# Liufeiran123/qwen2-audio-whisper-ggml

Measured on AMD Instinct MI355X. Metric: encoder audio-frames/sec (30 s clips) at 1/2/4/8 MI355X; MFMA util %, higher is better.
Workload: dtype q4_k x q8_k integer dots on fp16 MFMA (fp32 acc); 1 GPU; configs[2]: batch=64 30 s clips, Q4_K quantized weights, 1xMI355X per rank; model=qwen2-audio-encoder L32 D1280 H20 F5120 (synthetic weights), weights=q4_k, clips_per_gpu=64, global_batch=64, seq_len=3000, parallelism=dp1

## Files before the change

### include/q2a_encoder.h

```cpp
#ifndef Q2A_ENCODER_H
#define Q2A_ENCODER_H

#include <stddef.h>
#include <stdint.h>

#ifdef __cplusplus
extern "C" {
#endif

typedef struct q2a_engine q2a_engine;

typedef enum {
    Q2A_OK = 0,
    Q2A_ERR_IO = -1,
    Q2A_ERR_FORMAT = -2,
    Q2A_ERR_HIP = -3,
    Q2A_ERR_ARG = -4,
    Q2A_ERR_OOM = -5,
    Q2A_ERR_UNSUPPORTED = -6
} q2a_status;

#define Q2A_CLIP_ENCODED 0
#define Q2A_CLIP_SKIPPED 1
#define Q2A_CLIP_FAILED 2
// ... 66 lines not shown
                          int n_clips, int offset_ms, float * out_host, int32_t * status);
int q2a_group_setup_times(const q2a_group * g, double * pack_s, double * broadcast_s, double * open_s, int64_t * blob_bytes);

enum {
    Q2A_PROF_MEL = 0, Q2A_PROF_CONV1, Q2A_PROF_CONV2, Q2A_PROF_LN, Q2A_PROF_GEMM_QKV, Q2A_PROF_ATTN,
    Q2A_PROF_QUANT, Q2A_PROF_GEMM_O, Q2A_PROF_GEMM_FC1, Q2A_PROF_GEMM_FC2, Q2A_PROF_POOL, Q2A_PROF_CLASSES
};
int q2a_profile_enable(q2a_engine * e, int on);
int q2a_profile_enable_mask(q2a_engine * e, unsigned mask);
int q2a_profile_read(q2a_engine * e, double * ms, int64_t * counts, int n, int reset);

int q2a_test_linear(q2a_engine * e, int layer, int which, const float * x_dev, int M, float * y_dev, void * stream);
int q2a_test_block(q2a_engine * e, int layer, float * x_dev, int n_clips, void * stream);
int q2a_test_block_taps(q2a_engine * e, int layer, float * x_dev, int n_clips, void * const * taps, void * stream);
int q2a_test_frontend(q2a_engine * e, const float * pcm_dev, int64_t pcm_stride, const int32_t * n_samples, int n_clips,
                      float * x_dev, void * stream);
int q2a_test_pool_ln(q2a_engine * e, const float * x_dev, int n_clips, float * out_dev, void * stream);
int q2a_test_fc1_path(q2a_engine * e, int path);
int q2a_test_attention(q2a_engine * e, const float * q_dev, const float * k_dev, const float * v_dev, int n_clips,
                       float * out_dev, void * stream);
int q2a_test_attention_len(q2a_engine * e, const float * q_dev, const float * k_dev, const float * v_dev, int n_clips,
                           const int32_t * key_len, float * out_dev, void * stream);
int q2a_test_block_len(q2a_engine * e, int layer, float * x_dev, int n_clips, const int32_t * key_len, void * stream);

typedef struct q2a_projector q2a_projector;
q2a_projector * q2a_projector_open(const char * path, int device);
void q2a_projector_close(q2a_projector * p);
int q2a_projector_get_dims(const q2a_projector * p, int * d_in, int * d_out, int * wtype);
int q2a_projector_apply(q2a_projector * p, const float * x_dev, int64_t rows, float * y_dev, void * stream);

#ifdef __cplusplus
}
#endif
#endif
```

### qwen2-audio-whisper-ggml_amd/csrc/q2a_attn.hip

```cpp
#include "q2a_internal.h"

#include <cstddef>
#include <cstdlib>
#include <cstring>

namespace {

typedef _Float16 half8 __attribute__((ext_vector_type(8)));
typedef _Float16 half4 __attribute__((ext_vector_type(4)));
typedef short short8_t __attribute__((ext_vector_type(8)));
typedef float f16v __attribute__((ext_vector_type(16)));
typedef float f4v_t __attribute__((ext_vector_type(4)));
typedef __bf16 bf8 __attribute__((ext_vector_type(8)));
typedef __attribute__((address_space(3))) void * lds_ptr_t;

template <bool BF>
__device__ __forceinline__ f16v mma32(half8 a, half8 b, f16v c) {
    if constexpr (BF) return __builtin_amdgcn_mfma_f32_32x32x16_bf16(__builtin_bit_cast(bf8, a), __builtin_bit_cast(bf8, b), c, 0, 0, 0);
    else return __builtin_amdgcn_mfma_f32_32x32x16_f16(a, b, c, 0, 0, 0);
}
template <bool BF>
__device__ __forceinline__ _Float16 to16(float v) {
    if constexpr (BF) return __builtin_bit_cast(_Float16, (__bf16) v);
    else return (_Float16) v;
}


constexpr int KT = 64;
template <bool SW> struct attn_lds;
template <> struct attn_lds<false> {
    static constexpr int KROW = 144, VROW = 136;
    static __device__ __forceinline__ int k(int, int ch) { return ch << 4; }
    static __device__ __forceinline__ int v(int, int c8) { return c8 << 3; }
};
template <> struct attn_lds<true> {
// ... 27 lines not shown
}
constexpr int KS = 32;
__device__ __forceinline__ half2_t rem_pair(float p0, float p1, half2_t h) {
    half2_t r;
    asm("v_fma_mixlo_f16 %0, %1, -1.0, %2 op_sel_hi:[1,0,0]" : "=v"(r) : "v"(h), "v"(p0));
    asm("v_fma_mixhi_f16 %0, %1, -1.0, %2 op_sel:[1,0,0] op_sel_hi:[1,0,0]" : "+v"(r) : "v"(h), "v"(p1));
    return r;
}
__device__ __forceinline__ f4v_t mma16(half8 a, half8 b, f4v_t c) {
    return __builtin_amdgcn_mfma_f32_16x16x32_f16(a, b, c, 0, 0, 0);
}
__device__ __forceinline__ float max_lane16(float x) {
    const auto r = __builtin_amdgcn_permlane16_swap(__float_as_uint(x), __float_as_uint(x), false, false);
    return fmaxf(__uint_as_float(r[0]), __uint_as_float(r[1]));
}
__device__ __forceinline__ float sum_lane16(float x) {
    const auto r = __builtin_amdgcn_permlane16_swap(__float_as_uint(x), __float_as_uint(x), false, false);
    return __uint_as_float(r[0]) + __uint_as_float(r[1]);
}
__device__ __forceinline__ float sum_lane32(float x) {
    const auto r = __builtin_amdgcn_permlane32_swap(__float_as_uint(x), __float_as_uint(x), false, false);
    return __uint_as_float(r[0]) + __uint_as_float(r[1]);
}
template <bool VR, int NQB, bool KL = false>
__global__ __launch_bounds__(256, 3) void k_attn_t(const q2a_attn_args p) {
    static_assert(NQB == 1 || NQB == 2, "16 or 32 queries per wave");
    static_assert(!KL || VR, "key lengths: row-major V only (the V^T image's columns are not clamped)");
    constexpr int QWG = 64 * NQB;
    constexpr int KROW = 128, VROW = 64;
    constexpr int KIMG = KS * KROW, VIMG = 64 * VROW;
    constexpr int STAGE = 2 * KIMG + 2 * VIMG;
    __shared__ __attribute__((aligned(16))) char ldsA[STAGE];
    __shared__ __attribute__((aligned(16))) char ldsB[STAGE];
    __shared__ __attribute__((aligned(16))) char ldsC[STAGE];
    const int tid = threadIdx.x, lane = tid & 63, wave = __builtin_amdgcn_readfirstlane(tid >> 6);
    const int T = p.T, D = p.D;
    const int nq = (T + QWG - 1) / QWG, total = (int) gridDim.x;
    const int L = (int) blockIdx.x;
    const int w = (total & 7) ? L : (L & 7) * (total >> 3) + (L >> 3);
    const int qt = w % nq, h = (w / nq) % p.H, clip = w / (nq * p.H);
    const int q0 = qt * QWG + wave * 16 * NQB;
    const int64_t rowbase = (int64_t) clip * T;
    const int c16 = lane & 15, g = lane >> 4;
    int Tk = T;
    if constexpr (KL) {
        Tk = min(max(p.key_len[clip], 1), T);
        if (qt * QWG >= Tk) {
#pragma unroll
            for (int qb = 0; qb < NQB; ++qb) {
                const int q = q0 + 16 * qb + c16;
// ... 288 lines not shown
        for (int qb = 0; qb < NQB; ++qb) rebase(s0, qb, true);
        exps(s0, ex);
        splat(init);
    }
    for (int t = 0; t < ntiles; t += 3) {
        iter(ldsB, ldsA, ldsC, t);
        if (t + 1 >= ntiles) break;
        iter(ldsC, ldsB, ldsA, t + 1);
        if (t + 2 >= ntiles) break;
        iter(ldsA, ldsC, ldsB, t + 2);
    }

#pragma unroll
    for (int qb = 0; qb < NQB; ++qb) {
        const float l_tot = sum_lane32(sum_lane16(l_run[qb]));
        const float inv = 1.0f / l_tot;
        const int q = q0 + 16 * qb + c16;
        if (q < T) {
            const int64_t orow = (rowbase + q) * D + h * 64;
#pragma unroll
            for (int db = 0; db < 4; ++db) {
                const int d = 16 * db + 4 * g;
                f4v_t v = o[qb][db] * inv;
                if (p.outH) {
                    asm volatile("" : "+v"(v));
                    const half4 hv = {(_Float16) v[0], (_Float16) v[1], (_Float16) v[2], (_Float16) v[3]};
                    *(half4 *) (p.outH + orow + d) = hv;
                } else {
                    *(float4 *) (p.outF + orow + d) = make_float4(v[0], v[1], v[2], v[3]);
                }
            }
        }
    }
}

template <bool BF>
__global__ __launch_bounds__(512, 2) void k_attn_pp(const q2a_attn_args p) {
    constexpr float QL2E = BF ? L2E : 1.0f;
    typedef attn_lds<false> LY;
    constexpr int KROW = LY::KROW, VROW = LY::KROW;
    constexpr int KIMG = KT * KROW, VIMG = 64 * VROW;
    constexpr int NK = BF ? 1 : 2;
    constexpr int STAGE = NK * KIMG + VIMG;
    constexpr int NST = 3;
    constexpr int CH = (NK + 1) * 512;
    constexpr int CPT = CH / 512;
    __shared__ __attribute__((aligned(16))) char lds[NST * STAGE];
    const int tid = threadIdx.x, lane = tid & 63, wave = tid >> 6;
    const int grp = wave >> 2, gt = tid & 255;
    const int T = p.T, D = p.D;
    const int nq = (T + 255) / 256, total = (int) gridDim.x;
    const int L = (int) blockIdx.x;
    const int w = (total & 7) ? L : (L & 7) * (total >> 3) + (L >> 3);
    const int qt = w % nq, h = (w / nq) % p.H, clip = w / (nq * p.H);
    const int q0 = qt * 256 + wave * 32;
// ... 186 lines not shown
                    *(half4 *) (p.outH + orow + d) = hv;
                } else {
                    *(float4 *) (p.outF + orow + d) = make_float4(v0, v1, v2, v3);
                }
            }
    }
}
}

bool q2a_attention_wants_vlo() { return true; }

#ifndef Q2A_ATTN_LAUNCH
#define Q2A_ATTN_LAUNCH q2a_launch_attention
#endif
namespace {
hipError_t launch_attention(const q2a_attn_args & a, hipStream_t s) {
    if (a.D != a.H * 64 || a.TP < ((a.T + KT - 1) / KT) * KT) return hipErrorInvalidValue;
    if (a.key_len && (a.bf16 || !a.v_rows)) return hipErrorInvalidValue;
    if (a.bf16) {
        if (!a.outH) return hipErrorInvalidValue;
        hipLaunchKernelGGL(k_attn_pp<true>, dim3(((a.T + 255) / 256) * a.H * a.n_clips), dim3(512), 0, s, a);
    } else {
        if (!a.vtl) return hipErrorInvalidValue;
        const int n2 = ((a.T + 127) / 128) * a.H * a.n_clips;
        const bool narrow = n2 < q2a_cu_count();
        const dim3 grid(narrow ? ((a.T + 63) / 64) * a.H * a.n_clips : n2);
        if (a.key_len) {
            if (narrow) hipLaunchKernelGGL((k_attn_t<true, 1, true>), grid, dim3(256), 0, s, a);
            else hipLaunchKernelGGL((k_attn_t<true, 2, true>), grid, dim3(256), 0, s, a);
        } else if (a.v_rows) {
            if (narrow) hipLaunchKernelGGL((k_attn_t<true, 1>), grid, dim3(256), 0, s, a);
            else hipLaunchKernelGGL((k_attn_t<true, 2>), grid, dim3(256), 0, s, a);
        } else {
            if (narrow) hipLaunchKernelGGL((k_attn_t<false, 1>), grid, dim3(256), 0, s, a);
            else hipLaunchKernelGGL((k_attn_t<false, 2>), grid, dim3(256), 0, s, a);
        }
    }
    return hipGetLastError();
}
}

hipError_t Q2A_ATTN_LAUNCH(const q2a_attn_args & a, hipStream_t s) {
    q2a_attn_args b;
    memcpy(&b, &a, offsetof(q2a_attn_args, key_len));
    b.key_len = nullptr;
    return launch_attention(b, s);
}

hipError_t q2a_launch_attention_len(const q2a_attn_args & a, hipStream_t s) { return launch_attention(a, s); }
```

### qwen2-audio-whisper-ggml_amd/csrc/q2a_engine.hip

```cpp
#include "q2a_encoder.h"
#include "q2a_format.h"
#include "q2a_internal.h"

#include <algorithm>
#include <cmath>
#include <cerrno>
#include <cstdarg>
#include <cstdio>
#include <cstdlib>
#include <cstring>
#include <string>
#include <thread>
#include <vector>

namespace {

thread_local std::string g_err;

void set_err(const char * fmt, ...) {
    char buf[512];
    va_list ap;
    va_start(ap, fmt);
    vsnprintf(buf, sizeof(buf), fmt, ap);
    va_end(ap);
// ... 650 lines not shown
        size_t in_cap = 0, out_cap = 0;
        hipEvent_t h2d = nullptr, comp = nullptr, d2h = nullptr;
    };
    hipStream_t copy_stream = nullptr;
    host_buf hb[2];
    float * out_stage = nullptr;
    int32_t * meta = nullptr;
    int32_t * meta_host = nullptr;
    hipEvent_t meta_evt = nullptr;
    float * mel = nullptr;
    q2a_half * xc1 = nullptr;
    q2a_half * y1 = nullptr;
    float * X = nullptr;
    q2a_half * actD = nullptr;
    q2a_half * actF = nullptr;
    float * dyD = nullptr;
    float * dyF = nullptr;
    q2a_half * aextD = nullptr;
    q2a_half * aextF = nullptr;
    q2a_half *qh = nullptr, *ql = nullptr, *kh = nullptr, *kl = nullptr, *vt = nullptr;
    q2a_half * vtl = nullptr;
    float * attF = nullptr;
    float * hF = nullptr;
    float * part = nullptr;
    int2 * frange = nullptr;
    int TP = 0;
    int dy_ld = 0;
    bool force_encode = false;
    int fc1_path = 0;
    void * taps[4] = {nullptr, nullptr, nullptr, nullptr};

    bool prof = false;
    struct rec { int cls; hipEvent_t a, b; };
    std::vector<rec> pending;
    std::vector<hipEvent_t> pool;
    unsigned prof_mask = ~0u;
    double prof_ms[Q2A_PROF_CLASSES] = {};
    int64_t prof_n[Q2A_PROF_CLASSES] = {};

    template <class P> P g(int i) const { return (P) (blob + h.goff[i]); }
    template <class P> P lv(int l, int i) const { return (P) (blob + h.loff[l][i]); }
    const uint64_t * mat(int l, int w) const { return h.loff[l] + L_MAT0 + w * A_COUNT; }
};

namespace {

inline hipStream_t call_stream(const void * stream) { return (hipStream_t) stream; }

int engine_init(q2a_engine * e, int device) {
    int n = 0;
    HIP_TRY(hipGetDeviceCount(&n));
    if (device < 0 || device >= n) { set_err("device %d not available (%d devices)", device, n); return Q2A_ERR_HIP; }
    e->device = device;
    HIP_TRY(hipSetDevice(device));
    HIP_TRY(hipStreamCreateWithFlags(&e->stream, hipStreamNonBlocking));
    HIP_TRY(hipEventCreateWithFlags(&e->meta_evt, hipEventDisableTiming));
    return Q2A_OK;
}

int engine_adopt_header(q2a_engine * e) {
    if (const char * why = header_problem(e->h)) { set_err("%s", why); return Q2A_ERR_FORMAT; }
    e->d = dims_of(e->h.hp);
    e->wtype = e->h.wtype;
    e->blk = e->h.blk;
    e->f32 = e->wtype == Q2A_TYPE_F32;
    e->bf16 = e->h.act == Q2A_ACT_BF16;
    e->kx = e->f32 && !e->bf16 ? 3 : 1;
    e->gblk = e->bf16 ? Q2A_BLK_BF16 : e->blk;
    e->TP = ((e->d.T + 63) / 64) * 64;
    return Q2A_OK;
}

void free_ws(q2a_engine * e) {
    if (e->ws) (void) hipFree(e->ws);
    if (e->meta_host) (void) hipHostFree(e->meta_host);
    e->ws = nullptr; e->meta_host = nullptr;
    e->cap_clips = 0; e->ws_bytes = 0;
}

// ... 49 lines not shown
    HIP_TRY(hipSetDevice(e->device));
    HIP_TRY(hipDeviceSynchronize());
    if (e->ws) { (void) hipFree(e->ws); e->ws = nullptr; }
    if (e->meta_host) { (void) hipHostFree(e->meta_host); e->meta_host = nullptr; }
    const dims & d = e->d;
    const int64_t BT = (int64_t) B * d.T;
    const bool quant = e->blk != 0;
    size_t off = 0;
    auto take = [&](size_t bytes) { const size_t o = off; off += (bytes + 255) & ~size_t(255); return o; };
    const size_t o_meta = take((size_t) B * 5 * 4);
    const size_t o_mel = take((size_t) B * d.M * d.TM * 4);
    const size_t o_xc1 = take((size_t) B * (d.TM + 2) * 3 * d.M * 2);
    const size_t o_y1 = take((size_t) B * (d.TM + 1) * d.D * 2 * (e->f32 ? 2 : 1));
    const size_t o_X = take((size_t) BT * d.D * 4);
    const size_t o_actD = take((size_t) BT * d.D * 2 * e->kx);
    const size_t o_actF = take((size_t) BT * d.F * 2 * e->kx);
    const size_t o_qh = take((size_t) BT * d.D * 2);
    const size_t o_ql = take((size_t) BT * d.D * 2);
    const size_t o_kh = take((size_t) BT * d.D * 2);
    const size_t o_kl = take((size_t) BT * d.D * 2);
    const size_t o_vt = take((size_t) B * d.H * 64 * e->TP * 2);
    const bool vlo = !e->bf16 && q2a_attention_wants_vlo();
    const size_t o_vtl = vlo ? take((size_t) B * d.H * 64 * e->TP * 2) : 0;
    size_t o_dyD = 0, o_dyF = 0, o_aD = 0, o_aF = 0, o_att = 0, o_hF = 0, o_part = 0;
    const int64_t split_rows = std::min<int64_t>(BT, 32768);
    const bool split = !q2a_gemm_wide_tiles((int) split_rows, d.D, e->gblk);
    if (split) o_part = take((size_t) 4 * split_rows * d.D * 4);
    const int64_t MP = (BT + 255) / 256 * 256;
    e->dy_ld = (int) MP;
    if (quant) {
        o_dyD = take((size_t) MP * (d.D / 32) * 4);
        o_dyF = take((size_t) MP * (d.F / 32) * 4);
        o_aD = take((size_t) MP * (d.D / 256 + 1) * 16 * 2);
        o_aF = take((size_t) MP * (d.F / 256 + 1) * 16 * 2);
        o_att = take((size_t) BT * d.D * 4);
        o_hF = take((size_t) BT * d.F * 4);
    } else if (e->f32) {
        o_att = take((size_t) BT * d.D * 4);
    }
    void * ws = nullptr;
    if (hipMalloc(&ws, off) != hipSuccess) {
        (void) hipGetLastError();
        set_err("workspace allocation of %.2f GB for %d clips failed", off / 1e9, B);
        return Q2A_ERR_OOM;
    }
    HIP_TRY(hipMemsetAsync(ws, 0, off, e->stream));
    HIP_TRY(hipHostMalloc((void **) &e->meta_host, (size_t) B * 5 * 4, hipHostMallocDefault));
    uint8_t * b = (uint8_t *) ws;
    e->ws = ws; e->ws_bytes = off; e->cap_clips = B;
    e->meta = (int32_t *) (b + o_meta);
    e->mel = (float *) (b + o_mel);
    e->xc1 = (q2a_half *) (b + o_xc1);
    e->y1 = (q2a_half *) (b + o_y1);
    e->X = (float *) (b + o_X);
    e->actD = (q2a_half *) (b + o_actD);
    e->actF = (q2a_half *) (b + o_actF);
    e->qh = (q2a_half *) (b + o_qh); e->ql = (q2a_half *) (b + o_ql);
    e->kh = (q2a_half *) (b + o_kh); e->kl = (q2a_half *) (b + o_kl);
    e->vt = (q2a_half *) (b + o_vt);
    e->vtl = vlo ? (q2a_half *) (b + o_vtl) : nullptr;
    e->part = split ? (float *) (b + o_part) : nullptr;
    if (quant) {
        e->dyD = (float *) (b + o_dyD); e->dyF = (float *) (b + o_dyF);
        e->aextD = (q2a_half *) (b + o_aD); e->aextF = (q2a_half *) (b + o_aF);
        e->attF = (float *) (b + o_att); e->hF = (float *) (b + o_hF);
    } else if (e->f32) {
        e->attF = (float *) (b + o_att);
    }
    HIP_TRY(hipStreamSynchronize(e->stream));
    return Q2A_OK;
}

q2a_gemm_args gemm_base(const q2a_engine * e, int l, int which, const q2a_half * A, int M) {
    q2a_gemm_args a;
    memset(&a, 0, sizeof(a));
    int N, K;
    mat_dims(e->d, which, N, K);
    const uint64_t * m = e->mat(l, which);
    a.A = A; a.lda = (int64_t) K * e->kx; a.a_rpg = M; a.a_gstride = 0; a.a_step = 1;
    a.W = (const q2a_half *) (e->blob + m[A_W]); a.ldw = (int64_t) K * e->kx;
    a.M = M; a.N = N; a.K = K * e->kx;
    a.gelu_tab = e->g<const uint16_t *>(G_GELU);
    a.gelu_c = e->g<const uint16_t *>(G_GELU_C);
    a.T = e->d.T; a.D = e->d.D; a.H = e->d.H; a.TP = e->TP;
    if (e->blk) {
        a.nblk = K / e->blk;
        a.dx = (const float *) (e->blob + m[A_DX]);
        a.dy = K == e->d.D ? e->dyD : e->dyF;
// ... 20 lines not shown
    do {                                                                              \
        q2a_engine::rec r_{cls, nullptr, nullptr};                                    \
        const bool on_ = (e)->prof && (((e)->prof_mask >> (cls)) & 1);                 \
        if (on_) { r_.a = prof_event(e); r_.b = prof_event(e); (void) hipEventRecord(r_.a, s); } \
        hipError_t e_ = (call);                                                       \
        if (e_ != hipSuccess) {                                                       \
            set_err("%s: %s", #call, hipGetErrorString(e_));                        \
            return Q2A_ERR_HIP;                                                       \
        }                                                                             \
        if (on_) { (void) hipEventRecord(r_.b, s); (e)->pending.push_back(r_); }      \
    } while (0)

int ln_mode(const q2a_engine * e) { return e->bf16 ? 4 : e->f32 ? 3 : e->blk == 0 ? 0 : e->blk == 256 ? 1 : 2; }

#define LAUNCH(x)                                                                     \
    do {                                                                              \
        hipError_t e_ = (x);                                                          \
        if (e_ != hipSuccess) {                                                       \
            set_err("%s: %s", #x, hipGetErrorString(e_));                           \
            return Q2A_ERR_HIP;                                                       \
        }                                                                             \
    } while (0)

int run_block(q2a_engine * e, int l, int B, hipStream_t s, const int32_t * key_len = nullptr) {
    const dims & d = e->d;
    const int M = B * d.T;
    const int mode = ln_mode(e);
    auto tap = [&](int i, const q2a_half * src, int K) -> hipError_t {
        if (!e->taps[i]) return hipSuccess;
        return hipMemcpyAsync(e->taps[i], src, (size_t) M * K * e->kx * 2, hipMemcpyDeviceToDevice, s);
    };
    q2a_ln_args ln{e->X, M, d.D, e->lv<const float *>(l, L_LN1W), e->lv<const float *>(l, L_LN1B), mode, e->actD, e->dyD, e->aextD, e->dy_ld};
    PLAUNCH(e, s, Q2A_PROF_LN, q2a_launch_layernorm(ln, s));
    LAUNCH(tap(0, e->actD, d.D));
    {
        q2a_gemm_args a = gemm_base(e, l, 0, e->actD, M);
        a.bias = e->lv<const float *>(l, L_BQKV);
        a.qh = e->qh; a.ql = e->ql; a.kh = e->kh; a.kl = e->kl; a.vt = e->vt; a.vtl = e->vtl;
        a.v_rows = e->bf16 ? 0 : 1;
        a.qscale = (1.0f / sqrtf((float) (d.D / d.H))) * (e->bf16 ? 1.0f : Q2A_LOG2E);
        PLAUNCH(e, s, Q2A_PROF_GEMM_QKV, q2a_launch_gemm(a, Q2A_EPI_QKV, e->gblk, s));
    }
    {
        q2a_attn_args at{e->qh, e->ql, e->kh, e->kl, e->vt, B, d.T, d.D, d.H, e->TP, nullptr, nullptr, e->bf16 ? 1 : 0};
        at.vtl = e->vtl;
        at.v_rows = e->bf16 ? 0 : 1;
        at.key_len = key_len;
        if (mode == 0 || mode == 4) at.outH = e->actD; else at.outF = e->attF;
        if (key_len) PLAUNCH(e, s, Q2A_PROF_ATTN, q2a_launch_attention_len(at, s));
        else PLAUNCH(e, s, Q2A_PROF_ATTN, q2a_launch_attention(at, s));
        if (mode == 3) {
            const int64_t n = (int64_t) M * d.D;
            PLAUNCH(e, s, Q2A_PROF_QUANT, launch_split3(e->attF, e->actD, d.D, n, s));
        } else if (mode == 1 || mode == 2) {
            q2a_quant_args qa{e->attF, nullptr, M, d.D, mode, e->actD, e->dyD, e->aextD, e->dy_ld};
            PLAUNCH(e, s, Q2A_PROF_QUANT, q2a_launch_quant_act(qa, s));
        }
    }
    LAUNCH(tap(1, e->actD, d.D));
    {
        q2a_gemm_args a = gemm_base(e, l, 1, e->actD, M);
        a.bias = e->lv<const float *>(l, L_BO);
        a.outF = e->X; a.ldo = d.D;
        a.part = e->part; a.split_stride = (int64_t) M * d.D;
        PLAUNCH(e, s, Q2A_PROF_GEMM_O, q2a_launch_gemm(a, Q2A_EPI_RESID, e->gblk, s));
    }
    q2a_ln_args ln2{e->X, M, d.D, e->lv<const float *>(l, L_LN2W), e->lv<const float *>(l, L_LN2B), mode, e->actD, e->dyD, e->aextD, e->dy_ld};
    PLAUNCH(e, s, Q2A_PROF_LN, q2a_launch_layernorm(ln2, s));
    LAUNCH(tap(2, e->actD, d.D));
    {
        q2a_gemm_args a = gemm_base(e, l, 2, e->actD, M);
        a.bias = e->lv<const float *>(l, L_B1);
        if (mode == 0 || mode == 3 || mode == 4) {
            a.outH = e->actF; a.ldo = (int64_t) d.F * e->kx; a.o_rpg = M; a.o_gstride = 0; a.o_off = 0;
            a.o_dup = mode == 3 ? 2 * d.F : 0;
            PLAUNCH(e, s, Q2A_PROF_GEMM_FC1, q2a_launch_gemm(a, Q2A_EPI_GELU_H, e->gblk, s));
        } else if (mode == 1 && q2a_gemm_wide_tiles(M, d.F, e->blk) &&
// ... 676 lines not shown
    const int64_t n = (int64_t) n_clips * d.T * d.D;
    const dim3 g((unsigned) ((n + 255) / 256)), b(256);
    hipLaunchKernelGGL(k_split_hilo, g, b, 0, s, q, e->qh, e->ql, n, Q2A_LOG2E);
    hipLaunchKernelGGL(k_split_hilo, g, b, 0, s, k, e->kh, e->kl, n, 1.0f);
    hipLaunchKernelGGL(k_split_hilo, g, b, 0, s, v, e->vt, e->vtl, n, 1.0f);
    LAUNCH(hipGetLastError());
    q2a_attn_args at{e->qh, e->ql, e->kh, e->kl, e->vt, n_clips, d.T, d.D, d.H, e->TP, nullptr, out};
    at.vtl = e->vtl;
    at.v_rows = 1;
    at.key_len = with_len ? e->meta + 4 * n_clips : nullptr;
    if (with_len) LAUNCH(q2a_launch_attention_len(at, s));
    else LAUNCH(q2a_launch_attention(at, s));
    return Q2A_OK;
}

int q2a_test_attention(q2a_engine * e, const float * q, const float * k, const float * v, int n_clips, float * out,
                       void * stream) {
    return test_attention_impl(e, q, k, v, n_clips, nullptr, false, out, stream);
}

int q2a_test_attention_len(q2a_engine * e, const float * q, const float * k, const float * v, int n_clips,
                           const int32_t * key_len, float * out, void * stream) {
    return test_attention_impl(e, q, k, v, n_clips, key_len, true, out, stream);
}

struct q2a_projector {
    int device = 0;
    hipStream_t stream = nullptr;
    int d_in = 0, d_out = 0, wtype = 0, blk = 0;
    void * wdev = nullptr;
    uint64_t off[A_COUNT] = {};
    float * bias = nullptr;
    void * ws = nullptr;
    size_t ws_bytes = 0;
    const uint16_t * gelu = nullptr;
};

q2a_projector * q2a_projector_open(const char * path, int device) {
    char err[256] = {0};
    q2a_model_file * mf = q2a_model_file_read(path, err, sizeof(err));
    if (!mf) { set_err("projector %s: %s", path ? path : "(null)", err); return nullptr; }
    const q2a_tensor_desc * wt = q2a_model_file_find(mf, "multi_modal_projector.linear.weight");
    const q2a_tensor_desc * bt = q2a_model_file_find(mf, "multi_modal_projector.linear.bias");
    auto fail = [&](int code, const char * msg) -> q2a_projector * {
        set_err("projector %s: %s", path, msg);
        q2a_model_file_free(mf);
// ... 108 lines not shown
```

### qwen2-audio-whisper-ggml_amd/csrc/q2a_internal.h

```cpp
#pragma once

#include <hip/hip_runtime.h>
#include <stdint.h>

typedef _Float16 q2a_half;

extern "C" void q2a_internal_set_error(const char * msg);
struct q2a_engine;
extern "C" int q2a_internal_engine_blob(const q2a_engine * e, const void ** blob, int64_t * bytes, int * device);

enum q2a_epi {
    Q2A_EPI_QKV = 0,
    Q2A_EPI_RESID = 1,
    Q2A_EPI_GELU_H = 2,
    Q2A_EPI_CONV2 = 3,
    Q2A_EPI_GELU_F = 4,
    Q2A_EPI_STORE_F = 5,
    Q2A_EPI_GELU_Q8K = 6,
    Q2A_EPI_PRE_H = 7,
};

constexpr int Q2A_GELU_C_HALF = 0x4901;
constexpr int Q2A_GELU_C_BYTES = 5 * 16384;
static_assert(2 * Q2A_GELU_C_HALF * 2 <= Q2A_GELU_C_BYTES, "compact GELU table size");
// ... 58 lines not shown
int q2a_gemm_resid_ksplit(int M, int N, int K, int blk);
int q2a_gemm_kq_ksplit(int M, int N, int K, int blk);
constexpr int Q2A_BLK_BF16 = 1;
constexpr int Q2A_BLK_EXACT = 2;
hipError_t q2a_launch_gemm(const q2a_gemm_args & a, int epi, int blk, hipStream_t s);
bool q2a_gemm_wide_tiles(int M, int N, int blk);
int q2a_cu_count();
bool q2a_gemm_pipe8(const q2a_gemm_args & a, int blk);

struct q2a_attn_args {
    const q2a_half *qh, *ql, *kh, *kl, *vt;
    int n_clips, T, D, H, TP;
    q2a_half * outH;
    float * outF;
    int bf16;
    const q2a_half * vtl;
    int v_rows;
    const int32_t * key_len;
};
constexpr float Q2A_LOG2E = 1.4426950408889634f;
hipError_t q2a_launch_attention(const q2a_attn_args & a, hipStream_t s);
hipError_t q2a_launch_attention_len(const q2a_attn_args & a, hipStream_t s);
bool q2a_attention_wants_vlo();

struct q2a_mel_args {
    const float * pcm;
    int64_t pcm_stride;
    const int32_t * n_samples;
    const int32_t * seek;
    int n_clips;
    int n_mel, n_bins;
    int n_frames_win;
    int max_frames;
    const float * filters;
    const float * tab;
    const int2 * frange;
    float * mel;
    int32_t * clip_max;
    q2a_half * xc1;
    int xc_f32;
};
hipError_t q2a_launch_mel(const q2a_mel_args & a, hipStream_t s);
hipError_t q2a_launch_filter_ranges(const float * filters, int n_mel, int n_bins, int2 * out, hipStream_t s);

struct q2a_ln_args {
    const float * X;
// ... 41 lines not shown
```

### qwen2-audio-whisper-ggml_amd/csrc/q2a_quant.h

```cpp
#pragma once
#include "q2a_internal.h"

namespace {

template <int CTRL>
__device__ __forceinline__ uint32_t dpp_u(uint32_t v) {
    return (uint32_t) __builtin_amdgcn_mov_dpp((int) v, CTRL, 0xF, 0xF, false);
}
constexpr int DPP_ROR8 = 0x128, DPP_ROR4 = 0x124, DPP_ROR12 = 0x12C, DPP_XOR2 = 0x4E, DPP_XOR1 = 0xB1;

__device__ __forceinline__ float wave_max_f(float x) {
    x = fmaxf(x, __uint_as_float(dpp_u<DPP_ROR8>(__float_as_uint(x))));
    x = fmaxf(x, __uint_as_float(dpp_u<DPP_ROR4>(__float_as_uint(x))));
    x = fmaxf(x, __uint_as_float(dpp_u<DPP_XOR2>(__float_as_uint(x))));
    x = fmaxf(x, __uint_as_float(dpp_u<DPP_XOR1>(__float_as_uint(x))));
    const auto r = __builtin_amdgcn_permlane16_swap(__float_as_uint(x), __float_as_uint(x), false, false);
    x = fmaxf(__uint_as_float(r[0]), __uint_as_float(r[1]));
    const auto t = __builtin_amdgcn_permlane32_swap(__float_as_uint(x), __float_as_uint(x), false, false);
    return fmaxf(__uint_as_float(t[0]), __uint_as_float(t[1]));
}

__device__ __forceinline__ float first_max_value(float amax, float local_first, bool has, int lane, int group_lanes) {
    const unsigned long long m = __ballot(has);
    const int g0 = lane & ~(group_lanes - 1);
// ... 16 lines not shown
    float d = 1.f;
    if (amax != 0.f) {
        const float iscale = -127.f / mx;
        for (int e = 0; e < 4; ++e) q[e] = min(127, (int) rintf(iscale * vv[e]));
        d = 1 / iscale;
    }
    typedef _Float16 h4_t __attribute__((ext_vector_type(4)));
    *(h4_t *) codes = h4_t{(_Float16) (float) q[0], (_Float16) (float) q[1], (_Float16) (float) q[2], (_Float16) (float) q[3]};
    if (lane == 0) *dy_out = d;
    int s = q[0] + q[1] + q[2] + q[3];
    s += (int) dpp_u<DPP_XOR1>((uint32_t) s);
    s += (int) dpp_u<DPP_XOR2>((uint32_t) s);
    s += (int) dpp_u<DPP_ROR12>((uint32_t) s);
    if ((lane & 7) == 0) {
        const int j = lane >> 3;
        const int hi = (s >= 0) ? (s >> 6) : -((-s + 63) >> 6);
        const int lo = s - 64 * hi;
        aext[2 * j + 0] = (_Float16) (float) hi;
        aext[2 * j + 1] = (_Float16) (float) lo;
    }
}


__device__ __forceinline__ void quant_q8k_row16c(const float (&v)[16], int sub, q2a_half * codes, bool st, float & d_out,
                                                 int & s_out) {
    float lm = v[15];
#pragma unroll
    for (int e = 14; e >= 0; --e) lm = fabsf(v[e]) >= fabsf(lm) ? v[e] : lm;
    float amax = fabsf(lm);
    amax = fmaxf(amax, __uint_as_float(dpp_u<DPP_ROR8>(__float_as_uint(amax))));
    amax = fmaxf(amax, __uint_as_float(dpp_u<DPP_ROR4>(__float_as_uint(amax))));
    amax = fmaxf(amax, __uint_as_float(dpp_u<DPP_XOR2>(__float_as_uint(amax))));
    amax = fmaxf(amax, __uint_as_float(dpp_u<DPP_XOR1>(__float_as_uint(amax))));
    const int lane = __builtin_amdgcn_mbcnt_hi(~0u, __builtin_amdgcn_mbcnt_lo(~0u, 0u));
    const float mx = first_max_value(amax, lm, fabsf(lm) == amax, lane, 16);
    typedef float f2_t __attribute__((ext_vector_type(2)));
    float q[16];
    float d = 1.f;
    if (amax != 0.f) {
        const float iscale = -127.f / mx;
        const f2_t is2 = {iscale, iscale};
#pragma unroll
        for (int e = 0; e < 16; e += 2) {
            const f2_t y = is2 * f2_t{v[e], v[e + 1]};
            q[e] = rintf(y[0]);
            q[e + 1] = rintf(y[1]);
        }
        d = 1 / iscale;
    } else {
#pragma unroll
        for (int e = 0; e < 16; ++e) q[e] = 0.f;
    }
    typedef _Float16 h8_t __attribute__((ext_vector_type(8)));
    h8_t c0, c1;
#pragma unroll
    for (int e = 0; e < 8; ++e) { c0[e] = (_Float16) q[e]; c1[e] = (_Float16) q[8 + e]; }
    if (st) {
        *(h8_t *) codes = c0;
        *(h8_t *) (codes + 8) = c1;
    }
    f2_t s2 = {0.f, 0.f};
#pragma unroll
    for (int e = 0; e < 16; e += 2) s2 = s2 + f2_t{q[e], q[e + 1]};
    int s = (int) (s2[0] + s2[1]);
    s += (int) dpp_u<DPP_XOR1>((uint32_t) s);
    d_out = d;
    s_out = s;
}

// ... 84 lines not shown
```

### qwen2-audio-whisper-ggml_amd/q2a/__init__.py

```python
from __future__ import annotations

import ctypes as C
import os

import numpy as np

PKG_DIR = os.path.dirname(os.path.dirname(os.path.abspath(__file__)))
LIB_PATH = os.environ.get("Q2A_LIB_PATH") or os.path.join(PKG_DIR, "lib", "libq2a.so")
HOST_LIB_PATH = os.path.join(PKG_DIR, "lib", "libq2a_host.so")
TOOL_PATH = os.path.join(PKG_DIR, "bin", "q2a_tool")

EXPORTS = (
    "q2a_last_error", "q2a_open", "q2a_pack_model", "q2a_free_host_blob", "q2a_open_device_blob", "q2a_close",
    "q2a_get_info", "q2a_reserve", "q2a_encode_device", "q2a_encode_host", "q2a_pcm_to_mel",
    "q2a_encode_host_ex", "q2a_test_linear", "q2a_test_block", "q2a_test_block_taps", "q2a_test_attention", "q2a_test_fc1_path",
    "q2a_test_frontend", "q2a_test_pool_ln",
    "q2a_projector_open", "q2a_projector_close", "q2a_projector_get_dims", "q2a_projector_apply",
    "q2a_pack_model_compact", "q2a_blob_device_size", "q2a_expand_blob",
    "q2a_device_count", "q2a_group_open", "q2a_group_close", "q2a_group_size", "q2a_group_engine", "q2a_group_split",
    "q2a_group_encode_host", "q2a_group_setup_times", "q2a_group_open_with", "q2a_whisper_context_engine",
    "q2a_valid_lengths", "q2a_encode_device_padded", "q2a_encode_host_padded", "q2a_test_attention_len",
    "q2a_test_block_len",
)

CLIP_ENCODED, CLIP_SKIPPED, CLIP_FAILED = 0, 1, 2


class Q2AError(RuntimeError):
    pass


class Info(C.Structure):
    _fields_ = [("n_audio_ctx", C.c_int32), ("n_audio_state", C.c_int32), ("n_audio_head", C.c_int32),
                ("n_audio_layer", C.c_int32), ("n_mels", C.c_int32), ("wtype", C.c_int32), ("n_out", C.c_int32),
                ("device", C.c_int32), ("weight_bytes", C.c_int64), ("workspace_bytes", C.c_int64),
                ("act", C.c_int32), ("reserved", C.c_int32)]


ACT_REFERENCE = 0
ACT_BF16 = 1


_lib = None


# ... 33 lines not shown
        L.q2a_test_block.argtypes = [vp, C.c_int, vp, C.c_int, vp]
        L.q2a_test_block_taps.argtypes = [vp, C.c_int, vp, C.c_int, C.POINTER(vp), vp]
        L.q2a_test_attention.argtypes = [vp, vp, vp, vp, C.c_int, vp, vp]
        for name, at in (("q2a_test_fc1_path", [vp, C.c_int]), ("q2a_test_frontend", [vp, vp, C.c_int64, i32p, C.c_int, vp, vp]),
                         ("q2a_test_pool_ln", [vp, vp, C.c_int, vp, vp])):
            if hasattr(L, name):
                getattr(L, name).argtypes = at
        if hasattr(L, "q2a_group_open"):
            L.q2a_group_open.restype = vp
            L.q2a_group_open.argtypes = [C.c_char_p, i32p, C.c_int, C.c_int]
            L.q2a_group_open_with.restype = vp
            L.q2a_group_open_with.argtypes = [vp, i32p, C.c_int]
            L.q2a_group_close.argtypes = [vp]
            L.q2a_group_size.argtypes = [vp]
            L.q2a_group_engine.restype = vp
            L.q2a_group_engine.argtypes = [vp, C.c_int]
            L.q2a_group_split.argtypes = [C.c_int, C.c_int, C.c_int, i32p, i32p]
            L.q2a_group_encode_host.argtypes = [vp, C.POINTER(vp), i32p, i32p, C.c_int, C.c_int, vp, i32p]
            L.q2a_group_setup_times.argtypes = [vp, C.POINTER(C.c_double), C.POINTER(C.c_double),
                                                C.POINTER(C.c_double), C.POINTER(C.c_int64)]
        for name, at in (("q2a_encode_device_padded", [vp, vp, C.c_int64, i32p, i32p, i32p, C.c_int, vp, i32p, i32p, vp]),
                         ("q2a_encode_host_padded", [vp, C.POINTER(vp), i32p, i32p, i32p, C.c_int, vp, i32p, i32p]),
                         ("q2a_test_attention_len", [vp, vp, vp, vp, C.c_int, i32p, vp, vp]),
                         ("q2a_test_block_len", [vp, C.c_int, vp, C.c_int, i32p, vp])):
            if hasattr(L, name):
                getattr(L, name).argtypes = at
        L.q2a_projector_open.restype = vp
        L.q2a_projector_open.argtypes = [C.c_char_p, C.c_int]
        L.q2a_projector_close.argtypes = [vp]
        L.q2a_projector_get_dims.argtypes = [vp, i32p, i32p, i32p]
        L.q2a_projector_apply.argtypes = [vp, vp, C.c_int64, vp, vp]
        _lib = L
    return _lib


def _check(rc):
    if rc != 0:
        err = Q2AError(f"q2a error {rc}: {lib().q2a_last_error().decode()}")
        err.rc = rc
        raise err


class Engine:

    def __init__(self, model_path: str | None = None, device: int = 0, device_blob: int | None = None,
                 blob_size: int | None = None, act: int = ACT_REFERENCE):
        L = lib()
# ... 124 lines not shown
        ns = np.ascontiguousarray(n_samples, dtype=np.int32)
        _check(lib().q2a_test_frontend(self.h, C.c_void_p(pcm_ptr), C.c_int64(pcm_stride),
                                       ns.ctypes.data_as(C.POINTER(C.c_int32)), len(ns), C.c_void_p(x_ptr),
                                       C.c_void_p(stream) if stream else None))

    def test_pool_ln(self, x_ptr, n_clips, out_ptr, stream=None):
        _check(lib().q2a_test_pool_ln(self.h, C.c_void_p(x_ptr), n_clips, C.c_void_p(out_ptr),
                                      C.c_void_p(stream) if stream else None))

    def test_fc1_path(self, path):
        _check(lib().q2a_test_fc1_path(self.h, path))

    def test_attention(self, q_ptr, k_ptr, v_ptr, n_clips, out_ptr, stream=None):
        _check(lib().q2a_test_attention(self.h, C.c_void_p(q_ptr), C.c_void_p(k_ptr), C.c_void_p(v_ptr), n_clips,
                                        C.c_void_p(out_ptr), C.c_void_p(stream) if stream else None))

    def test_attention_len(self, q_ptr, k_ptr, v_ptr, n_clips, key_len, out_ptr, stream=None):
        kl = np.ascontiguousarray(key_len, dtype=np.int32)
        assert len(kl) == n_clips
        _check(lib().q2a_test_attention_len(self.h, C.c_void_p(q_ptr), C.c_void_p(k_ptr), C.c_void_p(v_ptr), n_clips,
                                            kl.ctypes.data_as(C.POINTER(C.c_int32)), C.c_void_p(out_ptr),
                                            C.c_void_p(stream) if stream else None))

    def test_block_len(self, layer, x_ptr, n_clips, key_len, stream=None):
        kl = np.ascontiguousarray(key_len, dtype=np.int32)
        assert len(kl) == n_clips
        _check(lib().q2a_test_block_len(self.h, layer, C.c_void_p(x_ptr), n_clips,
                                        kl.ctypes.data_as(C.POINTER(C.c_int32)), C.c_void_p(stream) if stream else None))


_host_lib = None


def valid_lengths(n_samples: int, offset_ms: int = 0, n_audio_ctx: int = 1500) -> tuple[int, int]:
    global _host_lib
    if _host_lib is None:
        if not os.path.exists(HOST_LIB_PATH):
            raise Q2AError(f"{HOST_LIB_PATH} not built; run `make -C {PKG_DIR} host`")
        _host_lib = C.CDLL(HOST_LIB_PATH)
        _host_lib.q2a_valid_lengths.argtypes = [C.c_int, C.c_int, C.c_int, C.POINTER(C.c_int32), C.POINTER(C.c_int32)]
    a, b = C.c_int32(), C.c_int32()
    rc = _host_lib.q2a_valid_lengths(n_samples, offset_ms, n_audio_ctx, C.byref(a), C.byref(b))
    if rc != 0:
        err = Q2AError(f"q2a error {rc}: invalid arguments to q2a_valid_lengths")
        err.rc = rc
        raise err
# ... 116 lines not shown
```

Baseline: 886,000 audio-frames/s.

## Fuse Q8_K activation quantization into the attention epilogue via last-head-arrival counters

The attention kernel gains a Q8 variant that writes fp32 output with buffer stores. Each group of four heads shares a 256-wide Q8_K block, so per query tile and head group an atomic counter picks the last arriving workgroup, and that workgroup quantizes the tile into codes, scales and aext. This removes the separate quant_act launch and its full reread of the attention output. It adds atomics, an agent-scope acquire fence and tail work done by one workgroup per group. It also adds a test entry point and an env switch to fall back to the separate path.

```diff
diff --git a/include/q2a_encoder.h b/include/q2a_encoder.h
--- a/include/q2a_encoder.h
+++ b/include/q2a_encoder.h
@@ -112,6 +112,8 @@
 int q2a_test_attention_len(q2a_engine * e, const float * q_dev, const float * k_dev, const float * v_dev, int n_clips,
                            const int32_t * key_len, float * out_dev, void * stream);
 int q2a_test_block_len(q2a_engine * e, int layer, float * x_dev, int n_clips, const int32_t * key_len, void * stream);
+int q2a_test_attention_q8k(q2a_engine * e, const float * q_dev, const float * k_dev, const float * v_dev, int n_clips,
+                           int fused, void * codes_dev, float * dy_dev, void * aext_dev, void * stream);
 
 typedef struct q2a_projector q2a_projector;
 q2a_projector * q2a_projector_open(const char * path, int device);
diff --git a/qwen2-audio-whisper-ggml_amd/csrc/q2a_attn.hip b/qwen2-audio-whisper-ggml_amd/csrc/q2a_attn.hip
--- a/qwen2-audio-whisper-ggml_amd/csrc/q2a_attn.hip
+++ b/qwen2-audio-whisper-ggml_amd/csrc/q2a_attn.hip
@@ -1,4 +1,5 @@
 #include "q2a_internal.h"
+#include "q2a_quant.h"
 
 #include <cstddef>
 #include <cstdlib>
@@ -11,6 +12,7 @@
 typedef short short8_t __attribute__((ext_vector_type(8)));
 typedef float f16v __attribute__((ext_vector_type(16)));
 typedef float f4v_t __attribute__((ext_vector_type(4)));
+typedef uint32_t u4v_t __attribute__((ext_vector_type(4)));
 typedef __bf16 bf8 __attribute__((ext_vector_type(8)));
 typedef __attribute__((address_space(3))) void * lds_ptr_t;
 
@@ -84,10 +86,14 @@
     const auto r = __builtin_amdgcn_permlane32_swap(__float_as_uint(x), __float_as_uint(x), false, false);
     return __uint_as_float(r[0]) + __uint_as_float(r[1]);
 }
-template <bool VR, int NQB, bool KL = false>
-__global__ __launch_bounds__(256, 3) void k_attn_t(const q2a_attn_args p) {
+struct attn_q8k_kargs : q2a_attn_args { q2a_attn_q8k_args x; };
+template <bool Q8> struct attn_kargs { typedef q2a_attn_args type; };
+template <> struct attn_kargs<true> { typedef attn_q8k_kargs type; };
+template <bool VR, int NQB, bool KL = false, bool Q8 = false>
+__global__ __launch_bounds__(256, 3) void k_attn_t(const typename attn_kargs<Q8>::type p) {
     static_assert(NQB == 1 || NQB == 2, "16 or 32 queries per wave");
     static_assert(!KL || VR, "key lengths: row-major V only (the V^T image's columns are not clamped)");
+    static_assert(!Q8 || (VR && NQB == 2 && !KL), "the Q8_K hand-off: the wide row-major grid without key lengths");
     constexpr int QWG = 64 * NQB;
     constexpr int KROW = 128, VROW = 64;
     constexpr int KIMG = KS * KROW, VIMG = 64 * VROW;
@@ -422,7 +428,11 @@
             for (int db = 0; db < 4; ++db) {
                 const int d = 16 * db + 4 * g;
                 f4v_t v = o[qb][db] * inv;
-                if (p.outH) {
+                if constexpr (Q8) {
+                    const __amdgpu_buffer_rsrc_t rs = __builtin_amdgcn_make_buffer_rsrc(
+                        (void *) (p.outF + rowbase * D + h * 64), 0, (T * D - h * 64) * 4, 0x00020000);
+                    __builtin_amdgcn_raw_buffer_store_b128(__builtin_bit_cast(u4v_t, v), rs, (q * D + d) * 4, 0, 16);
+                } else if (p.outH) {
                     asm volatile("" : "+v"(v));
                     const half4 hv = {(_Float16) v[0], (_Float16) v[1], (_Float16) v[2], (_Float16) v[3]};
                     *(half4 *) (p.outH + orow + d) = hv;
@@ -431,6 +441,63 @@
                 }
             }
         }
+    }
+    if constexpr (Q8) {
+        asm volatile("s_waitcnt vmcnt(0)" ::: "memory");
+        __syncthreads();
+        uint32_t * last = (uint32_t *) ldsA;
+        const int hg = h >> 2;
+        if (tid == 0) {
+            typedef __attribute__((address_space(1))) uint32_t gu32;
+            gu32 * cnt = (gu32 *) (p.x.counters + ((int64_t) clip * nq + qt) * (p.H >> 2) + hg);
+            const uint32_t k = __hip_atomic_fetch_add(cnt, 1u, __ATOMIC_RELAXED, __HIP_MEMORY_SCOPE_AGENT);
+            if (k == 3) {
+                __hip_atomic_store(cnt, 0u, __ATOMIC_RELAXED, __HIP_MEMORY_SCOPE_AGENT);
+                __builtin_amdgcn_fence(__ATOMIC_ACQUIRE, "agent");
+                asm volatile("s_waitcnt vmcnt(0)" ::: "memory");
+            }
+            *last = k;
+        }
+        __syncthreads();
+        if (*last != 3) return;
+        const int r0 = qt * QWG, nrows = min(QWG, T - r0);
+        const int64_t m0 = rowbase + r0;
+        const int sub = lane & 15, grp = lane >> 4;
+        const int64_t blk0 = (int64_t) hg * p.x.dy_ld + m0;
+        float * sd = (float *) ldsB;
+        constexpr int NI = QWG / 16, PH = 4;
+#pragma unroll
+        for (int i0 = 0; i0 < NI; i0 += PH) {
+            float y[PH][16];
+#pragma unroll
+            for (int i = 0; i < PH; ++i) {
+                const int r = min(16 * (i0 + i) + 4 * wave + grp, nrows - 1);
+#pragma unroll
+                for (int j = 0; j < 4; ++j) {
+                    const float4 f = *(const float4 *) (p.outF + (m0 + r) * D + hg * 256 + 16 * sub + 4 * j);
+                    y[i][4 * j] = f.x; y[i][4 * j + 1] = f.y; y[i][4 * j + 2] = f.z; y[i][4 * j + 3] = f.w;
+                }
+            }
+#pragma unroll
+            for (int i = 0; i < PH; ++i) {
+                const int rb = 16 * (i0 + i) + 4 * wave;
+                if (rb < nrows) {
+                    const int r = rb + grp;
+                    const bool ok = r < nrows;
+                    float dq;
+                    int bs;
+                    quant_q8k_row16c<true>(y[i], sub, p.x.codes + (m0 + min(r, nrows - 1)) * D + hg * 256 + 16 * sub, ok, dq, bs);
+                    if (ok && sub == 0) sd[r] = dq;
+                    if (ok && (sub & 1) == 0) {
+                        const int hi = (bs >= 0) ? (bs >> 6) : -((-bs + 63) >> 6);
+                        const int lo = bs - 64 * hi;
+                        *(half2_t *) (p.x.aext + (blk0 + r) * 16 + sub) = half2_t{(_Float16) (float) hi, (_Float16) (float) lo};
+                    }
+                }
+            }
+        }
+        __syncthreads();
+        if (tid < nrows) p.x.dy[blk0 + tid] = sd[tid];
     }
 }
 
@@ -663,9 +730,8 @@
         hipLaunchKernelGGL(k_attn_pp<true>, dim3(((a.T + 255) / 256) * a.H * a.n_clips), dim3(512), 0, s, a);
     } else {
         if (!a.vtl) return hipErrorInvalidValue;
-        const int n2 = ((a.T + 127) / 128) * a.H * a.n_clips;
-        const bool narrow = n2 < q2a_cu_count();
-        const dim3 grid(narrow ? ((a.T + 63) / 64) * a.H * a.n_clips : n2);
+        const bool narrow = !q2a_attention_wide(a.n_clips, a.T, a.H);
+        const dim3 grid(((a.T + (narrow ? 63 : 127)) / (narrow ? 64 : 128)) * a.H * a.n_clips);
         if (a.key_len) {
             if (narrow) hipLaunchKernelGGL((k_attn_t<true, 1, true>), grid, dim3(256), 0, s, a);
             else hipLaunchKernelGGL((k_attn_t<true, 2, true>), grid, dim3(256), 0, s, a);
@@ -689,3 +755,19 @@
 }
 
 hipError_t q2a_launch_attention_len(const q2a_attn_args & a, hipStream_t s) { return launch_attention(a, s); }
+
+bool q2a_attention_wide(int n_clips, int T, int H) { return ((T + 127) / 128) * H * n_clips >= q2a_cu_count(); }
+
+int64_t q2a_attention_q8k_counters(int n_clips, int T, int D) { return (int64_t) n_clips * ((T + 127) / 128) * (D / 256); }
+
+hipError_t q2a_launch_attention_q8k(const q2a_attn_args & a, const q2a_attn_q8k_args & x, hipStream_t s) {
+    if (a.D != a.H * 64 || a.D % 256 != 0 || a.TP < ((a.T + KT - 1) / KT) * KT) return hipErrorInvalidValue;
+    if (a.bf16 || !a.v_rows || !a.vtl || a.outH || !a.outF || a.key_len) return hipErrorInvalidValue;
+    if (!x.codes || !x.dy || !x.aext || !x.counters || x.dy_ld < a.n_clips * a.T) return hipErrorInvalidValue;
+    if ((int64_t) a.T * a.D * 4 > INT32_MAX || !q2a_attention_wide(a.n_clips, a.T, a.H)) return hipErrorInvalidValue;
+    attn_q8k_kargs k;
+    memcpy(static_cast<q2a_attn_args *>(&k), &a, sizeof(a));
+    k.x = x;
+    hipLaunchKernelGGL((k_attn_t<true, 2, false, true>), dim3(((a.T + 127) / 128) * a.H * a.n_clips), dim3(256), 0, s, k);
+    return hipGetLastError();
+}
diff --git a/qwen2-audio-whisper-ggml_amd/csrc/q2a_engine.hip b/qwen2-audio-whisper-ggml_amd/csrc/q2a_engine.hip
--- a/qwen2-audio-whisper-ggml_amd/csrc/q2a_engine.hip
+++ b/qwen2-audio-whisper-ggml_amd/csrc/q2a_engine.hip
@@ -696,6 +696,8 @@
     q2a_half * vtl = nullptr;
     float * attF = nullptr;
     float * hF = nullptr;
+    uint32_t * attn_cnt = nullptr;
+    bool attn_q8k_off = false;
     float * part = nullptr;
     int2 * frange = nullptr;
     int TP = 0;
@@ -729,6 +731,8 @@
     HIP_TRY(hipSetDevice(device));
     HIP_TRY(hipStreamCreateWithFlags(&e->stream, hipStreamNonBlocking));
     HIP_TRY(hipEventCreateWithFlags(&e->meta_evt, hipEventDisableTiming));
+    const char * sep = getenv("Q2A_ATTN_Q8K_SEPARATE");
+    e->attn_q8k_off = sep && *sep && strcmp(sep, "0") != 0;
     return Q2A_OK;
 }
 
@@ -824,7 +828,7 @@
     const size_t o_vt = take((size_t) B * d.H * 64 * e->TP * 2);
     const bool vlo = !e->bf16 && q2a_attention_wants_vlo();
     const size_t o_vtl = vlo ? take((size_t) B * d.H * 64 * e->TP * 2) : 0;
-    size_t o_dyD = 0, o_dyF = 0, o_aD = 0, o_aF = 0, o_att = 0, o_hF = 0, o_part = 0;
+    size_t o_dyD = 0, o_dyF = 0, o_aD = 0, o_aF = 0, o_att = 0, o_hF = 0, o_part = 0, o_cnt = 0;
     const int64_t split_rows = std::min<int64_t>(BT, 32768);
     const bool split = !q2a_gemm_wide_tiles((int) split_rows, d.D, e->gblk);
     if (split) o_part = take((size_t) 4 * split_rows * d.D * 4);
@@ -837,6 +841,7 @@
         o_aF = take((size_t) MP * (d.F / 256 + 1) * 16 * 2);
         o_att = take((size_t) BT * d.D * 4);
         o_hF = take((size_t) BT * d.F * 4);
+        if (e->blk == 256) o_cnt = take((size_t) q2a_attention_q8k_counters(B, d.T, d.D) * 4);
     } else if (e->f32) {
         o_att = take((size_t) BT * d.D * 4);
     }
@@ -866,6 +871,7 @@
         e->dyD = (float *) (b + o_dyD); e->dyF = (float *) (b + o_dyF);
         e->aextD = (q2a_half *) (b + o_aD); e->aextF = (q2a_half *) (b + o_aF);
         e->attF = (float *) (b + o_att); e->hF = (float *) (b + o_hF);
+        e->attn_cnt = e->blk == 256 ? (uint32_t *) (b + o_cnt) : nullptr;
     } else if (e->f32) {
         e->attF = (float *) (b + o_att);
     }
@@ -932,6 +938,11 @@
         }                                                                             \
     } while (0)
 
+bool attn_writes_q8k(const q2a_engine * e, int B, bool with_len) {
+    return ln_mode(e) == 1 && !with_len && !e->attn_q8k_off && e->attn_cnt && e->d.D % 256 == 0 &&
+           q2a_attention_wide(B, e->d.T, e->d.H);
+}
+
 int run_block(q2a_engine * e, int l, int B, hipStream_t s, const int32_t * key_len = nullptr) {
     const dims & d = e->d;
     const int M = B * d.T;
@@ -957,12 +968,15 @@
         at.v_rows = e->bf16 ? 0 : 1;
         at.key_len = key_len;
         if (mode == 0 || mode == 4) at.outH = e->actD; else at.outF = e->attF;
-        if (key_len) PLAUNCH(e, s, Q2A_PROF_ATTN, q2a_launch_attention_len(at, s));
+        const bool q8k = attn_writes_q8k(e, B, key_len != nullptr);
+        const q2a_attn_q8k_args ax{e->actD, e->dyD, e->aextD, e->dy_ld, e->attn_cnt};
+        if (q8k) PLAUNCH(e, s, Q2A_PROF_ATTN, q2a_launch_attention_q8k(at, ax, s));
+        else if (key_len) PLAUNCH(e, s, Q2A_PROF_ATTN, q2a_launch_attention_len(at, s));
         else PLAUNCH(e, s, Q2A_PROF_ATTN, q2a_launch_attention(at, s));
         if (mode == 3) {
             const int64_t n = (int64_t) M * d.D;
             PLAUNCH(e, s, Q2A_PROF_QUANT, launch_split3(e->attF, e->actD, d.D, n, s));
-        } else if (mode == 1 || mode == 2) {
+        } else if ((mode == 1 || mode == 2) && !q8k) {
             q2a_quant_args qa{e->attF, nullptr, M, d.D, mode, e->actD, e->dyD, e->aextD, e->dy_ld};
             PLAUNCH(e, s, Q2A_PROF_QUANT, q2a_launch_quant_act(qa, s));
         }
@@ -1685,6 +1699,43 @@
 int q2a_test_attention_len(q2a_engine * e, const float * q, const float * k, const float * v, int n_clips,
                            const int32_t * key_len, float * out, void * stream) {
     return test_attention_impl(e, q, k, v, n_clips, key_len, true, out, stream);
+}
+
+int q2a_test_attention_q8k(q2a_engine * e, const float * q, const float * k, const float * v, int n_clips, int fused,
+                           void * codes, float * dy, void * aext, void * stream) {
+    if (!e || n_clips <= 0 || !codes || !dy || !aext || ln_mode(e) != 1) return Q2A_ERR_ARG;
+    HIP_TRY(hipSetDevice(e->device));
+    hipStream_t s = call_stream(stream);
+    int rc = reserve(e, n_clips);
+    if (rc) return rc;
+    const dims & d = e->d;
+    const int M = n_clips * d.T, MP = (M + 255) / 256 * 256, nb = d.D / 256;
+    const int64_t n = (int64_t) M * d.D;
+    const size_t ld = (size_t) e->dy_ld;
+    HIP_TRY(hipMemcpyAsync(e->actD, codes, (size_t) n * 2, hipMemcpyDeviceToDevice, s));
+    HIP_TRY(hipMemcpy2DAsync(e->dyD, ld * 4, dy, (size_t) MP * 4, (size_t) MP * 4, nb, hipMemcpyDeviceToDevice, s));
+    HIP_TRY(hipMemcpy2DAsync(e->aextD, ld * 32, aext, (size_t) MP * 32, (size_t) MP * 32, nb, hipMemcpyDeviceToDevice, s));
+    const dim3 g((unsigned) ((n + 255) / 256)), b(256);
+    hipLaunchKernelGGL(k_split_hilo, g, b, 0, s, q, e->qh, e->ql, n, Q2A_LOG2E);
+    hipLaunchKernelGGL(k_split_hilo, g, b, 0, s, k, e->kh, e->kl, n, 1.0f);
+    hipLaunchKernelGGL(k_split_hilo, g, b, 0, s, v, e->vt, e->vtl, n, 1.0f);
+    LAUNCH(hipGetLastError());
+    q2a_attn_args at{e->qh, e->ql, e->kh, e->kl, e->vt, n_clips, d.T, d.D, d.H, e->TP, nullptr, e->attF};
+    at.vtl = e->vtl;
+    at.v_rows = 1;
+    at.key_len = nullptr;
+    if (fused) {
+        const q2a_attn_q8k_args ax{e->actD, e->dyD, e->aextD, e->dy_ld, e->attn_cnt};
+        LAUNCH(q2a_launch_attention_q8k(at, ax, s));
+    } else {
+        LAUNCH(q2a_launch_attention(at, s));
+        q2a_quant_args qa{e->attF, nullptr, M, d.D, 1, e->actD, e->dyD, e->aextD, e->dy_ld};
+        LAUNCH(q2a_launch_quant_act(qa, s));
+    }
+    HIP_TRY(hipMemcpyAsync(codes, e->actD, (size_t) n * 2, hipMemcpyDeviceToDevice, s));
+    HIP_TRY(hipMemcpy2DAsync(dy, (size_t) MP * 4, e->dyD, ld * 4, (size_t) MP * 4, nb, hipMemcpyDeviceToDevice, s));
+    HIP_TRY(hipMemcpy2DAsync(aext, (size_t) MP * 32, e->aextD, ld * 32, (size_t) MP * 32, nb, hipMemcpyDeviceToDevice, s));
+    return Q2A_OK;
 }
 
 struct q2a_projector {
diff --git a/qwen2-audio-whisper-ggml_amd/csrc/q2a_internal.h b/qwen2-audio-whisper-ggml_amd/csrc/q2a_internal.h
--- a/qwen2-audio-whisper-ggml_amd/csrc/q2a_internal.h
+++ b/qwen2-audio-whisper-ggml_amd/csrc/q2a_internal.h
@@ -104,6 +104,16 @@
 hipError_t q2a_launch_attention(const q2a_attn_args & a, hipStream_t s);
 hipError_t q2a_launch_attention_len(const q2a_attn_args & a, hipStream_t s);
 bool q2a_attention_wants_vlo();
+bool q2a_attention_wide(int n_clips, int T, int H);
+struct q2a_attn_q8k_args {
+    q2a_half * codes;
+    float * dy;
+    q2a_half * aext;
+    int dy_ld;
+    uint32_t * counters;
+};
+int64_t q2a_attention_q8k_counters(int n_clips, int T, int D);
+hipError_t q2a_launch_attention_q8k(const q2a_attn_args & a, const q2a_attn_q8k_args & x, hipStream_t s);
 
 struct q2a_mel_args {
     const float * pcm;
diff --git a/qwen2-audio-whisper-ggml_amd/csrc/q2a_quant.h b/qwen2-audio-whisper-ggml_amd/csrc/q2a_quant.h
--- a/qwen2-audio-whisper-ggml_amd/csrc/q2a_quant.h
+++ b/qwen2-audio-whisper-ggml_amd/csrc/q2a_quant.h
@@ -62,6 +62,7 @@
 }
 
 
+template <bool PZ = false>
 __device__ __forceinline__ void quant_q8k_row16c(const float (&v)[16], int sub, q2a_half * codes, bool st, float & d_out,
                                                  int & s_out) {
     float lm = v[15];
@@ -85,6 +86,7 @@
             const f2_t y = is2 * f2_t{v[e], v[e + 1]};
             q[e] = rintf(y[0]);
             q[e + 1] = rintf(y[1]);
+            if constexpr (PZ) { q[e] += 0.f; q[e + 1] += 0.f; }
         }
         d = 1 / iscale;
     } else {
diff --git a/qwen2-audio-whisper-ggml_amd/q2a/__init__.py b/qwen2-audio-whisper-ggml_amd/q2a/__init__.py
--- a/qwen2-audio-whisper-ggml_amd/q2a/__init__.py
+++ b/qwen2-audio-whisper-ggml_amd/q2a/__init__.py
@@ -20,7 +20,7 @@
     "q2a_device_count", "q2a_group_open", "q2a_group_close", "q2a_group_size", "q2a_group_engine", "q2a_group_split",
     "q2a_group_encode_host", "q2a_group_setup_times", "q2a_group_open_with", "q2a_whisper_context_engine",
     "q2a_valid_lengths", "q2a_encode_device_padded", "q2a_encode_host_padded", "q2a_test_attention_len",
-    "q2a_test_block_len",
+    "q2a_test_block_len", "q2a_test_attention_q8k",
 )
 
 CLIP_ENCODED, CLIP_SKIPPED, CLIP_FAILED = 0, 1, 2
@@ -100,7 +100,8 @@
         for name, at in (("q2a_encode_device_padded", [vp, vp, C.c_int64, i32p, i32p, i32p, C.c_int, vp, i32p, i32p, vp]),
                          ("q2a_encode_host_padded", [vp, C.POINTER(vp), i32p, i32p, i32p, C.c_int, vp, i32p, i32p]),
                          ("q2a_test_attention_len", [vp, vp, vp, vp, C.c_int, i32p, vp, vp]),
-                         ("q2a_test_block_len", [vp, C.c_int, vp, C.c_int, i32p, vp])):
+                         ("q2a_test_block_len", [vp, C.c_int, vp, C.c_int, i32p, vp]),
+                         ("q2a_test_attention_q8k", [vp, vp, vp, vp, C.c_int, C.c_int, vp, vp, vp, vp])):
             if hasattr(L, name):
                 getattr(L, name).argtypes = at
         L.q2a_projector_open.restype = vp
@@ -271,6 +272,11 @@
                                             kl.ctypes.data_as(C.POINTER(C.c_int32)), C.c_void_p(out_ptr),
                                             C.c_void_p(stream) if stream else None))
 
+    def test_attention_q8k(self, q_ptr, k_ptr, v_ptr, n_clips, fused, codes_ptr, dy_ptr, aext_ptr, stream=None):
+        _check(lib().q2a_test_attention_q8k(self.h, C.c_void_p(q_ptr), C.c_void_p(k_ptr), C.c_void_p(v_ptr), n_clips,
+                                            int(fused), C.c_void_p(codes_ptr), C.c_void_p(dy_ptr), C.c_void_p(aext_ptr),
+                                            C.c_void_p(stream) if stream else None))
+
     def test_block_len(self, layer, x_ptr, n_clips, key_len, stream=None):
         kl = np.ascontiguousarray(key_len, dtype=np.int32)
         assert len(kl) == n_clips
```

Result: no change. 887,500 audio-frames/s (median of 5 runs) (+0.2%).
